# TritonDataCenter/binder

Hardware: AMD Instinct MI355X
Metric: dns_queries_per_sec (higher is better)
Workload: dtype n/a

## Files before the change

native/balancer/balancer_main.cpp:

```cpp
#include <arpa/inet.h>
#include <dirent.h>
#include <netinet/in.h>
#include <netinet/udp.h>
#include <signal.h>
#include <sys/epoll.h>
#include <sys/eventfd.h>
#include <sys/signalfd.h>
#include <sys/socket.h>
#include <sys/stat.h>
#include <sys/un.h>
#include <unistd.h>

#include <algorithm>
#include <cstdlib>
#include <cstring>
#include <map>
#include <unordered_map>
#include <chrono>
#include <memory>
#include <unordered_map>
#include <mutex>
#include <thread>
#include <set>
#include <string>
// ... 183 lines not shown
  private:
    void rescan();
    void connectBackend(Backend* be);
    void backendDown(Backend* be);
    void onBackendEvent(std::shared_ptr<Backend> be, uint32_t ev);
    void onBackendBell(std::shared_ptr<Backend> be);
    void serveBackend(Backend* be, bool fromRing);
    void offerShm(Backend* be);
    void dropShm(Backend* be);
    EventLoop::Park beforePark(bool park);
    void backendFlush(Backend* be);
    void flushToRing(Backend* be);
    Backend* pickBackend(const std::string& remoteIp);
    Backend* pickBackendFast(const struct sockaddr_storage& ss);
    Backend* chooseLeastLoaded();
    void onUdpReadable();
    Backend* routeFor(const struct sockaddr_storage& src);
    void handleUdpQuery(const uint8_t* dns, size_t dnsLen,
                        const struct sockaddr_storage& src,
                        int64_t expiry, Backend* be);
    void onTcpAccept();
    void onTcpClient(std::shared_ptr<TcpClient> c, uint32_t ev);
    void tcpClientFlush(TcpClient* c);
    void onStatsAccept();
    void sweep();
    Json snapshot() const;

    EventLoop* loop_;
    Logger log_;
    std::string host_;
    uint16_t port_;
// ... 3 lines not shown
    bool reusePort_ = false;
    int workerId_ = 0;
    int nWorkers_ = 1;

    int udpFd_ = -1, tcpFd_ = -1, statsFd_ = -1;
    std::map<std::string, std::shared_ptr<Backend>> backends_;
    std::map<int, std::shared_ptr<Backend>> backendsById_;
    std::map<std::string, int> remotes_;
    std::unordered_map<uint64_t, int> remotesFast_;
    std::map<int, std::shared_ptr<TcpClient>> tcpClients_;
    int nextBackendId_ = 1;
    int salvageDepth_ = 0;
    uint64_t udpQueries_ = 0, udpReplies_ = 0, drops_ = 0;
    uint64_t backendReads_ = 0, udpRxMsgs_ = 0;
    uint64_t shmDoorbells_ = 0, shmDrains_ = 0;

    static constexpr size_t kMaxRemotes = 262144;
    static constexpr size_t kMaxPending = 16384;
    static constexpr int64_t kReplyTtlMs = 3000;
    static constexpr int64_t kPingIntervalMs = 2000;
    static constexpr int64_t kPingTimeoutMs = 6000;

    static constexpr int kBatch = 128;
    static constexpr size_t kRxBufSz = 65536;
    std::vector<uint8_t> rxArena_ =
        std::vector<uint8_t>((size_t)kBatch * kRxBufSz);
    struct mmsghdr rxHdrs_[kBatch];
    struct iovec rxIovs_[kBatch];
    struct sockaddr_storage rxAddrs_[kBatch];
    char rxCtrl_[kBatch][CMSG_SPACE(sizeof(uint16_t))];
// ... 468 lines not shown
    if (be->fd >= 0 && be->rxShm) serveBackend(be.get(), true);
}

EventLoop::Park Balancer::beforePark(bool park) {
    EventLoop::Park out = EventLoop::Park::NoRings;
    for (auto& [id, be] : backendsById_) {
        if (!be->rxShm || be->fd < 0) continue;
        if (out == EventLoop::Park::NoRings) out = EventLoop::Park::Idle;
        if (park) {
            if (!be->shm.rx.park()) out = EventLoop::Park::Work;
        } else if (be->shm.rx.readable() != 0 || be->shm.rx.bad()) {
            serveBackend(be.get(), true);
            out = EventLoop::Park::Work;
        }
    }
    return out;
}

void Balancer::serveBackend(Backend* be, bool fromRing) {
    size_t got = 0;
    while (got < kMaxReadPerEvent) {
        if (fromRing) {
            size_t n = be->shm.rx.read(be->in.tail(kReadChunk), kReadChunk);
            if (n == 0) break;
            be->in.commit(n);
            got += n;
            backendReads_++;
            shmDrains_++;
            if (n < kReadChunk) break;
            continue;
// ... 203 lines not shown
    if (ss.ss_family == AF_INET) {
        const auto* sa = (const struct sockaddr_in*)&ss;
        inet_ntop(AF_INET, &sa->sin_addr, out, n);
        *port = ntohs(sa->sin_port);
        *family = 4;
        memcpy(addr16, &sa->sin_addr, 4);
    } else {
        const auto* sa = (const struct sockaddr_in6*)&ss;
        inet_ntop(AF_INET6, &sa->sin6_addr, out, n);
        *port = ntohs(sa->sin6_port);
        *family = 6;
        memcpy(addr16, &sa->sin6_addr, 16);
    }
}

void Balancer::onUdpReadable() {
    struct mmsghdr* hdrs = rxHdrs_;
    struct sockaddr_storage* addrs = rxAddrs_;

    while (true) {
        int n = recvmmsg(udpFd_, hdrs, kBatch, 0, nullptr);
        if (n <= 0) return;
        udpRxMsgs_ += (uint64_t)n;
        int64_t expiry = monotonicMillis() + kReplyTtlMs;
        Touched touched;
        for (int i = 0; i < n; ++i) {
            size_t seg = hdrs[i].msg_len;
            for (struct cmsghdr* cm = CMSG_FIRSTHDR(&hdrs[i].msg_hdr);
                 cm != nullptr;
                 cm = CMSG_NXTHDR(&hdrs[i].msg_hdr, cm)) {
                if (cm->cmsg_level == SOL_UDP &&
                    cm->cmsg_type == UDP_GRO) {
                    uint16_t g;
                    memcpy(&g, CMSG_DATA(cm), sizeof(g));
                    if (g > 0) seg = g;
                }
            }
            hdrs[i].msg_hdr.msg_namelen = sizeof(addrs[i]);
            hdrs[i].msg_hdr.msg_controllen = sizeof(rxCtrl_[i]);
            hdrs[i].msg_hdr.msg_flags = 0;
            Backend* be = routeFor(addrs[i]);
            const uint8_t* base = rxArena_.data() + (size_t)i * kRxBufSz;
            size_t total = hdrs[i].msg_len;
            for (size_t off = 0; off < total; off += seg) {
                size_t dnsLen = std::min(seg, total - off);
                handleUdpQuery(base + off, dnsLen, addrs[i], expiry, be);
            }
            if (be != nullptr) touch(touched, be);
        }
        flushTouched(touched);
        if (n < kBatch) return;
    }
}

void Balancer::handleUdpQuery(const uint8_t* dns, size_t dnsLen,
                              const struct sockaddr_storage& src,
                              int64_t expiry, Backend* be) {
    udpQueries_++;
    if (be == nullptr) {
        drops_++;
        return;
    }
    if (be->pendingCount > kMaxPending ||
        be->out.size() - be->outOff > (4u << 20)) {
        drops_++;
        return;
// ... 187 lines not shown
        r.set("backend", Json((int64_t)id));
        rms.push_back(std::move(r));
    }
    out.set("remotes", Json(std::move(rms)));
    out.set("udp_queries", Json((int64_t)udpQueries_));
    out.set("udp_replies", Json((int64_t)udpReplies_));
    out.set("drops", Json((int64_t)drops_));
    out.set("reply_runs", Json((int64_t)replyRuns_.runs()));
    out.set("reply_run_segments",
            Json((int64_t)replyRuns_.runSegments()));
    out.set("reply_singles", Json((int64_t)replyRuns_.singles()));
    out.set("backend_reads", Json((int64_t)backendReads_));
    out.set("udp_rx_msgs", Json((int64_t)udpRxMsgs_));
    out.set("shm_doorbells", Json((int64_t)shmDoorbells_));
    out.set("shm_drains", Json((int64_t)shmDrains_));
    return out;
}

void Balancer::onStatsAccept() {
    while (true) {
        int fd = accept4(statsFd_, nullptr, nullptr,
                         SOCK_CLOEXEC | SOCK_NONBLOCK);
        if (fd < 0) return;
        g_stats.publish(workerId_, snapshot().dump());
        std::map<std::string, Json> byPath;
        JsonArray remotes;
        int64_t udpQ = 0, udpR = 0, drops = 0;
        static const char* const kHot[] = {
            "reply_runs", "reply_run_segments", "reply_singles",
            "backend_reads", "udp_rx_msgs", "shm_doorbells",
            "shm_drains"};
        constexpr int kNHot = 7;
        int64_t hot[kNHot] = {0, 0, 0, 0, 0, 0, 0};
        JsonArray perWorker;
        int workers = 0;
        for (const std::string& frag : g_stats.all()) {
            auto parsed = Json::parse(frag);
            if (!parsed) continue;
            workers++;
            udpQ += parsed->get("udp_queries").asInt();
            udpR += parsed->get("udp_replies").asInt();
            drops += parsed->get("drops").asInt();
            Json pw = Json::object();
            pw.set("udp_queries", parsed->get("udp_queries"));
            pw.set("udp_replies", parsed->get("udp_replies"));
            pw.set("drops", parsed->get("drops"));
            for (int k = 0; k < kNHot; ++k) {
                hot[k] += parsed->get(kHot[k]).asInt();
// ... 178 lines not shown
```

native/common/loop.cpp:

```cpp
#include "loop.hpp"

#include <fcntl.h>
#include <sys/epoll.h>
#include <sys/eventfd.h>
#include <unistd.h>

#include <cstdio>
#include <cstring>
#include <stdexcept>

#include "log.hpp"

namespace bamd {

bool setNonBlocking(int fd) {
    int flags = fcntl(fd, F_GETFL, 0);
    if (flags < 0) return false;
    return fcntl(fd, F_SETFL, flags | O_NONBLOCK) == 0;
}

EventLoop::EventLoop() {
    epfd_ = epoll_create1(EPOLL_CLOEXEC);
    if (epfd_ < 0)
        throw std::runtime_error(std::string("epoll_create1: ") +
                                 strerror(errno));
    wakeFd_ = eventfd(0, EFD_NONBLOCK | EFD_CLOEXEC);
    if (wakeFd_ >= 0) {
        addFd(wakeFd_, EPOLLIN, [this](uint32_t) {
            uint64_t v;
            while (read(wakeFd_, &v, sizeof(v)) == sizeof(v)) {
            }
            std::vector<TimerCallback> tasks;
            {
                std::lock_guard<std::mutex> g(postMutex_);
                tasks.swap(posted_);
            }
            for (auto& t : tasks) t();
        });
    }
}
// ... 87 lines not shown
}

void EventLoop::runOnce(int64_t maxWaitMs) {
    std::unique_lock<std::mutex> lk;
    if (dispatchLock_ != nullptr)
        lk = std::unique_lock<std::mutex>(*dispatchLock_);
    if (!deferred_.empty()) {
        std::vector<TimerCallback> tasks;
        tasks.swap(deferred_);
        for (auto& t : tasks) t();
    }

    Park ring = beforePark_ ? beforePark_(false) : Park::NoRings;
    bool busy = ring == Park::Work;

    int64_t wait = nextTimerDelay();
    if (wait < 0 || wait > maxWaitMs) wait = maxWaitMs;
    if (ring == Park::NoRings) {
        hadWork_ = false;
    } else if (busy || hadWork_) {
        wait = 0;
    } else if (wait != 0 && beforePark_(true) == Park::Work) {
        wait = 0;
    }

    struct epoll_event evs[64];
    if (lk.owns_lock()) lk.unlock();
    int n = epoll_wait(epfd_, evs, 64, (int)wait);
    int waitErrno = errno;
    if (dispatchLock_ != nullptr) lk.lock();
    errno = waitErrno;
    hadWork_ = ring != Park::NoRings && (busy || n > 0);
    if (n < 0) {
        if (errno == EINTR) return;
        throw std::runtime_error(std::string("epoll_wait: ") +
                                 strerror(errno));
    }
    dispatching_ = true;
    for (int i = 0; i < n; ++i) {
        int fd = (int)(uint32_t)evs[i].data.u64;
        uint32_t gen = (uint32_t)(evs[i].data.u64 >> 32);
        auto it = fds_.find(fd);
        if (it == fds_.end()) continue;
        if (it->second.gen != gen) continue;
// ... 31 lines not shown
```

native/common/loop.hpp:

```cpp
#pragma once

#include <atomic>
#include <cstdint>
#include <functional>
#include <map>
#include <memory>
#include <mutex>
#include <queue>
#include <thread>
#include <vector>

namespace bamd {

class EventLoop {
  public:
    using FdCallback = std::function<void(uint32_t events)>;
    using TimerCallback = std::function<void()>;

    EventLoop();
    ~EventLoop();
    EventLoop(const EventLoop&) = delete;
    EventLoop& operator=(const EventLoop&) = delete;

    void addFd(int fd, uint32_t events, FdCallback cb);
// ... 3 lines not shown
    uint64_t addTimer(int64_t delayMs, TimerCallback cb);
    void cancelTimer(uint64_t id);

    void defer(TimerCallback cb);

    void postFromThread(TimerCallback cb);

    void run();
    void stop() { running_ = false; }
    bool running() const { return running_; }

    bool runUntil(const std::function<bool()>& pred, int64_t timeoutMs);

    void setDispatchLock(std::mutex* m) { dispatchLock_ = m; }

    enum class Park { NoRings, Idle, Work };
    using ParkHook = std::function<Park(bool park)>;
    void setBeforePark(ParkHook h) { beforePark_ = std::move(h); }

    bool inLoopThread() const {
        return loopThread_.load(std::memory_order_relaxed) ==
               std::this_thread::get_id();
    }

  private:
    void runOnce(int64_t maxWaitMs);
    void wake();
    void wakeIfForeign() {
        if (dispatchLock_ != nullptr && !inLoopThread()) wake();
    }
    int64_t nextTimerDelay() const;
    void fireTimers();

// ... 15 lines not shown
    }

    int epfd_;
    std::atomic<bool> running_{false};
    std::map<int, FdReg> fds_;
    std::vector<std::unique_ptr<FdCallback>> retired_;
    bool dispatching_ = false;
    uint32_t nextFdGen_ = 1;
    std::priority_queue<Timer, std::vector<Timer>, std::greater<Timer>> heap_;
    std::map<uint64_t, TimerCallback> timers_;
    uint64_t nextTimerId_ = 1;
    std::vector<TimerCallback> deferred_;
    ParkHook beforePark_;
    bool hadWork_ = false;

    int wakeFd_ = -1;
    std::mutex* dispatchLock_ = nullptr;
    std::atomic<std::thread::id> loopThread_{};
    std::mutex postMutex_;
    std::vector<TimerCallback> posted_;
};

bool setNonBlocking(int fd);

}
```

native/common/shmpipe.hpp:

```cpp
#pragma once

#include <fcntl.h>
#include <sys/mman.h>
#include <sys/stat.h>
#include <unistd.h>

#include <atomic>
#include <cstddef>
#include <cstdint>
#include <cstring>
#include <new>

namespace bamd::shm {

constexpr uint32_t kVersion = 1;
constexpr size_t kMinRing = 4096;
constexpr size_t kMaxRing = 64u << 20;
constexpr size_t kDefaultRing = 256u << 10;
constexpr size_t kDataOff = 4096;

struct RingCtl {
    alignas(64) std::atomic<uint64_t> tail;
    alignas(64) std::atomic<uint64_t> head;
    alignas(64) std::atomic<uint32_t> consumerParked;
// ... 10 lines not shown
inline size_t regionBytes(size_t cap) { return kDataOff + 2 * cap; }

inline void ringDoorbell(int efd) {
    uint64_t one = 1;
    ssize_t rv = ::write(efd, &one, sizeof(one));
    (void)rv;
}

class Producer {
  public:
    void attach(RingCtl* ctl, uint8_t* data, size_t cap) {
        ctl_ = ctl;
        data_ = data;
        cap_ = cap;
        tail_ = 0;
        lastHead_ = 0;
        bad_ = false;
    }
    bool bad() const { return bad_; }

    size_t write(const void* src, size_t len) {
        size_t room = space();
        if (len > room) len = room;
        if (len == 0) return 0;
        size_t off = (size_t)(tail_ & (cap_ - 1));
        size_t first = cap_ - off;
        if (first > len) first = len;
        memcpy(data_ + off, src, first);
        if (len > first)
            memcpy(data_, (const uint8_t*)src + first, len - first);
        tail_ += len;
        ctl_->tail.store(tail_, std::memory_order_release);
        return len;
    }

    bool consumerNeedsWake() {
        std::atomic_thread_fence(std::memory_order_seq_cst);
        if (ctl_->consumerParked.load(std::memory_order_relaxed) == 0)
            return false;
        return ctl_->consumerParked.exchange(
                   0, std::memory_order_acq_rel) != 0;
    }

    bool waitForSpace() {
        ctl_->producerWaiting.store(1, std::memory_order_relaxed);
        std::atomic_thread_fence(std::memory_order_seq_cst);
        if (space() == 0 && !bad_) return true;
        ctl_->producerWaiting.store(0, std::memory_order_relaxed);
// ... 4 lines not shown
    size_t space() {
        if (bad_) return 0;
        uint64_t head = ctl_->head.load(std::memory_order_acquire);
        if (head > tail_ || tail_ - head > cap_ || head < lastHead_) {
            bad_ = true;
            return 0;
        }
        lastHead_ = head;
        return cap_ - (size_t)(tail_ - head);
    }

    RingCtl* ctl_ = nullptr;
    uint8_t* data_ = nullptr;
    size_t cap_ = 0;
    uint64_t tail_ = 0;
    uint64_t lastHead_ = 0;
    bool bad_ = false;
};

class Consumer {
  public:
    void attach(RingCtl* ctl, const uint8_t* data, size_t cap) {
        ctl_ = ctl;
        data_ = data;
        cap_ = cap;
        head_ = 0;
        lastTail_ = 0;
        parked_ = false;
        bad_ = false;
    }
// ... 153 lines not shown
```

native/server/answertab.hpp:

```cpp
#pragma once

#include <cstdint>
#include <cstring>
#include <memory>

namespace bamd {

#ifdef BAMD_ANSWERTAB_TEST_HASH_MASK
inline uint64_t answertabTestHashMask = ~0ull;
#endif

class AnswerTable {
  public:
    static constexpr size_t kMaxKey = 255;
    static constexpr uint32_t kNone = 0xFFFFFFFFu;
    static constexpr size_t kMinSlots = 1024;
    static constexpr size_t kCompactMinDead = 1u << 20;
    static constexpr size_t kDefaultMaxArena = 256u << 20;

    explicit AnswerTable(size_t maxArena = kDefaultMaxArena,
                         size_t compactMinDead = kCompactMinDead)
        : maxArena_(maxArena), compactMinDead_(compactMinDead) {}

    static uint64_t hashKey(const void* key, size_t klen, uint8_t qtype) {
// ... 308 lines not shown
    memcpy(tab + 8 * n, head, headLen);
    size_t off = 0;
    for (size_t i = 0; i < n; ++i) {
        put16(tab + 8 * i, off);
        put16(tab + 8 * i + 2, seg1[i].n);
        if (seg1[i].n != 0) memcpy(segs + off, seg1[i].p, seg1[i].n);
        off += seg1[i].n;
        put16(tab + 8 * i + 4, off);
        put16(tab + 8 * i + 6, seg2[i].n);
        if (seg2[i].n != 0) memcpy(segs + off, seg2[i].p, seg2[i].n);
        off += seg2[i].n;
    }
    put16(body + 2, headLen + off);
}
inline size_t serviceMembers(const uint8_t* body) { return body[1]; }
inline size_t serviceAssemble(const uint8_t* body, const uint8_t* order,
                              uint8_t* dst) {
    size_t n = body[1];
    size_t headLen = get16(body + 4);
    const uint8_t* tab = body + 6;
    const uint8_t* head = tab + 8 * n;
    const uint8_t* segs = head + headLen;
    uint8_t* w = dst;
    memcpy(w, head, headLen);
    w += headLen;
    for (size_t i = 0; i < n; ++i) {
        const uint8_t* e = tab + 8 * order[i];
        size_t len = get16(e + 2);
        memcpy(w, segs + get16(e), len);
        w += len;
// ... 14 lines not shown
```

native/server/metrics.hpp:

```cpp
#pragma once

#include <atomic>
#include <cstdint>
#include <functional>
#include <map>
#include <memory>
#include <string>
#include <vector>

#include "../common/loop.hpp"

namespace bamd {

struct CounterShard {
    std::atomic<uint64_t> v{0};
    void bump() {
        v.store(v.load(std::memory_order_relaxed) + 1,
                std::memory_order_relaxed);
    }
    uint64_t read() const { return v.load(std::memory_order_relaxed); }
};
struct CounterFold {
    uint64_t seen = 0;
};

class Counter {
  public:
    void increment(const std::string& labels, uint64_t by = 1) {
        vals_[labels] += by;
    }
    uint64_t& slot(const std::string& labels) { return vals_[labels]; }
    void set(const std::string& labels, uint64_t v) {
        vals_[labels] = v;
    }
    const std::map<std::string, uint64_t>& values() const { return vals_; }
    void fold(const std::string& labels, const CounterShard& s,
              CounterFold& f) {
        uint64_t now = s.read();
        if (now != f.seen) vals_[labels] += now - f.seen;
        f.seen = now;
    }

  private:
    std::map<std::string, uint64_t> vals_;
};

class Histogram {
  public:
    Histogram();
    void observe(const std::string& labels, double v);

    struct Series;
    Series& seriesRef(const std::string& labels);
// ... 91 lines not shown
```

native/server/server.cpp:

```cpp
#include "server.hpp"

#include <arpa/inet.h>
#include <sched.h>
#include <sys/epoll.h>
#include <unistd.h>

#include <cstdio>
#include <cstdlib>
#include <cstring>
#include <fstream>

#include "../balancer/protocol.hpp"
#include "../common/probes.hpp"

namespace bamd {

using namespace dns;

void fillClientInfo(ClientInfo& ci, const struct sockaddr_storage& ss,
                    const char* family) {
    ci.family = family;
    if (ss.ss_family == AF_INET) {
        const auto* sa = (const struct sockaddr_in*)&ss;
        memcpy(ci.addr, &sa->sin_addr, 4);
// ... 26 lines not shown
    uint8_t head[bsock::kHeaderLen + 4];
    head[0] = bsock::kMagic;
    head[1] = bsock::FRAME_REPLY;
    head[2] = (uint8_t)plen;
    head[3] = (uint8_t)(plen >> 8);
    head[4] = (uint8_t)(plen >> 16);
    head[5] = (uint8_t)(plen >> 24);
    head[6] = (uint8_t)reqId_;
    head[7] = (uint8_t)(reqId_ >> 8);
    head[8] = (uint8_t)(reqId_ >> 16);
    head[9] = (uint8_t)(reqId_ >> 24);
    frames_->append((const char*)head, sizeof(head));
    start_ = frames_->size();
}

uint8_t* ReplySink::openWrite(size_t dnsLen) {
    if (vec_ != nullptr) {
        vec_->resize(dnsLen);
        return vec_->data();
    }
    constexpr size_t kHead = bsock::kHeaderLen + 4;
    size_t at = frames_->size();
    frames_->resize(at + kHead + dnsLen);
    uint8_t* h = (uint8_t*)frames_->data() + at;
    uint32_t plen = (uint32_t)(4 + dnsLen);
    h[0] = bsock::kMagic;
    h[1] = bsock::FRAME_REPLY;
    h[2] = (uint8_t)plen;
    h[3] = (uint8_t)(plen >> 8);
    h[4] = (uint8_t)(plen >> 16);
    h[5] = (uint8_t)(plen >> 24);
    h[6] = (uint8_t)reqId_;
    h[7] = (uint8_t)(reqId_ >> 8);
    h[8] = (uint8_t)(reqId_ >> 16);
    h[9] = (uint8_t)(reqId_ >> 24);
    start_ = at + kHead;
    return h + kHead;
}

DnsServer::DnsServer(EventLoop* loop, Logger log, ServerOptions opts,
                     Engine* engine, Collector* collector)
    : loop_(loop), log_(std::move(log)), opts_(std::move(opts)),
      engine_(engine), collector_(collector) {
    main_.loop = loop_;
    collector_->setBeforeExpose([this]() { foldShards(); });
    reqCounter_ = collector->counter("binder_requests_completed",
                                     "count of Binder requests completed");
    latHist_ = collector->histogram(
        "binder_request_latency_seconds",
        "total time to process Binder requests");
    sizeHist_ = collector->histogram("binder_response_size_bytes",
                                     "size in bytes of Binder responses");
    shmDoorbellCounter_ = collector->counter(
        "binder_balancer_shm_doorbells",
        "doorbells rung to wake a balancer across shared-memory rings");
    shmDrainCounter_ = collector->counter(
        "binder_balancer_shm_drains",
        "takes from a shared-memory query ring that returned data");

    const EngineConfig& cfg = engine_->config();
    if (!cfg.dnsDomain.empty()) dotDomain_ = "." + cfg.dnsDomain;
    dcSuffix_ = cfg.dnsDomain + "." + cfg.datacenterName;

    rxArena_.resize(kBatch * kInBuf);
    rxHdrs_.resize(kBatch);
    rxIovs_.resize(kBatch);
    rxAddrs_.resize(kBatch);
    txBufs_.resize(kBatch);
    txHdrs_.resize(kBatch);
    txIovs_.resize(kBatch);
    txAddrs_.resize(kBatch);
}

// ... 445 lines not shown
    static const std::string kA = "type=\"A\"";
    static const std::string kSrv = "type=\"SRV\"";
    auto fold = [this](ServeCtx& c) {
        reqCounter_->fold(kA, c.hits.cntA, c.folds.cntA);
        reqCounter_->fold(kSrv, c.hits.cntSrv, c.folds.cntSrv);
        latHist_->fold(kA, c.hits.latA, c.folds.latA);
        latHist_->fold(kSrv, c.hits.latSrv, c.folds.latSrv);
        sizeHist_->fold(kA, c.hits.sizeA, c.folds.sizeA);
        sizeHist_->fold(kSrv, c.hits.sizeSrv, c.folds.sizeSrv);
    };
    fold(main_);
    for (auto& c : pool_) fold(*c);
    auto foldShm = [this](ServeCtx& c) {
        shmDoorbellCounter_->fold("", c.shmDoorbells, c.shmDoorbellsFold);
        shmDrainCounter_->fold("", c.shmDrains, c.shmDrainsFold);
    };
    foldShm(main_);
    for (auto& c : pool_) foldShm(*c);
    if (queriesServed() != servedSlow_) {
        reqCounter_->slot(kA);
        reqCounter_->slot(kSrv);
        latHist_->seriesRef(kA);
        latHist_->seriesRef(kSrv);
        sizeHist_->seriesRef(kA);
        sizeHist_->seriesRef(kSrv);
    }
}

void DnsServer::serveHit(ServeCtx& ctx, const uint8_t* body, bool isSrv,
                         const uint8_t* data, ReplySink& out) {
    const size_t total = answerbody::total(body);
    uint8_t* w = out.openWrite(total);
    if (answerbody::kind(body) == answerbody::kWire) {
        memcpy(w, answerbody::wireReply(body), total);
    } else {
        size_t n = answerbody::serviceMembers(body);
        uint8_t order[answerbody::kMaxMembers];
        for (size_t i = 0; i < n; ++i) order[i] = (uint8_t)i;
        for (size_t i = n; i > 1;) {
            --i;
            size_t j = ctx.rng() % (i + 1);
            std::swap(order[i], order[j]);
        }
        answerbody::serviceAssemble(body, order, w);
    }
    w[0] = data[0];
    w[1] = data[1];
    w[2] = (uint8_t)(w[2] | (data[2] & 0x01));

    countFast(ctx, isSrv, total);
    BAMD_PROBE2("op-req-done", total, 0);
}

bool DnsServer::fastPath(ServeCtx& ctx, const uint8_t* data, size_t len,
                         bool udp, const ClientInfo& ci, ReplySink& out) {
    if (log_.enabled(LogLevel::Debug)) return false;
    FastQuery q;
    if (!parseFast(data, len, q)) return false;
    bool memo = answersOn();
    if (memo) {
        q.hash = answerHash(q);
        const uint8_t* body = ctx.answers.find(q.hash, q.isSrv ? 33 : 1,
                                               q.name, q.nlen);
// ... 1042 lines not shown
```

native/server/server.hpp:

```cpp
#pragma once

#include <netinet/in.h>
#include <sys/socket.h>
#include <sys/un.h>

#include <atomic>
#include <functional>
#include <random>
#include <map>
#include <memory>
#include <mutex>
#include <string>
#include <thread>
#include <vector>

#include "../common/log.hpp"
#include "../common/loop.hpp"
#include "../common/shmpipe.hpp"
#include "../engine/engine.hpp"
#include "answertab.hpp"
#include "framebuf.hpp"
#include "metrics.hpp"

namespace bamd {
// ... 20 lines not shown
    uint8_t ipFamily = 0;
    uint16_t port = 0;
    const char* family = "udp";

    const char* address(char (&buf)[48]) const;
};

class ReplySink {
  public:
    explicit ReplySink(std::vector<uint8_t>* v) : vec_(v) {}
    ReplySink(std::string* frames, uint32_t reqId)
        : frames_(frames), reqId_(reqId) {}

    void open(size_t dnsLen);
    uint8_t* openWrite(size_t dnsLen);
    void append(const uint8_t* p, size_t n) {
        if (vec_ != nullptr)
            vec_->insert(vec_->end(), p, p + n);
        else
            frames_->append((const char*)p, n);
    }
    uint8_t* dns() {
        return vec_ != nullptr ? vec_->data()
                               : (uint8_t*)frames_->data() + start_;
    }
    size_t dnsLen() const {
        return vec_ != nullptr ? vec_->size() : frames_->size() - start_;
    }
    std::vector<uint8_t>* vec() { return vec_; }

// ... 131 lines not shown
        CounterFold cntA, cntSrv;
        Histogram::Fold latA, latSrv, sizeA, sizeSrv;
    };
    void countFast(ServeCtx& ctx, bool isSrv, size_t bytes);
    void foldShards();

    struct alignas(64) ServeCtx {
        AnswerTable answers;
        std::mt19937 rng{std::random_device{}()};
        HitShards hits;
        EventLoop* loop = nullptr;
        std::map<int, std::shared_ptr<BalConn>> balConns;
        std::vector<BalConn*> shmConns;
        CounterShard shmDoorbells, shmDrains;
        CounterFold shmDoorbellsFold, shmDrainsFold;
        bool pooled = false;

        std::atomic<uint64_t> inboxSeq{0};
        uint64_t inboxSeen = 0;
        std::mutex inboxMu;
        std::vector<std::string> inbox;

        HitFolds folds;

        std::unique_ptr<EventLoop> ownLoop;
        std::thread thread;
    };
    void postInvalidate(ServeCtx& ctx, std::string_view domain);
    void drainInbox(ServeCtx& ctx) {
        if (ctx.inboxSeq.load(std::memory_order_acquire) != ctx.inboxSeen)
// ... 47 lines not shown
    void sweepIdleTcp();
    void balFlush(ServeCtx& ctx, BalConn* c);
    void closeTcp(TcpConn* c);
    void closeBal(ServeCtx& ctx, BalConn* c);

    EventLoop* loop_;
    Logger log_;
    ServerOptions opts_;
    Engine* engine_;
    Collector* collector_;
    RecursionIface* recursion_ = nullptr;

    Counter* reqCounter_ = nullptr;
    Counter* shmDoorbellCounter_ = nullptr;
    Counter* shmDrainCounter_ = nullptr;
    Histogram* latHist_ = nullptr;
    Histogram* sizeHist_ = nullptr;

    int udpFd_ = -1;
    int tcpFd_ = -1;
    int balFd_ = -1;
    uint16_t boundPort_ = 0;
    uint64_t servedSlow_ = 0;

    std::map<int, std::shared_ptr<TcpConn>> tcpConns_;

    static constexpr int kBatch = 64;
    static constexpr size_t kInBuf = 4096;
    std::vector<uint8_t> rxArena_;
    std::vector<struct mmsghdr> rxHdrs_;
// ... 13 lines not shown
```

Before: 24.16 million.

## Skip redundant epoll polls in busy loops and poll UDP from ring hook

The event loop now skips the epoll_wait call on busy rounds for up to a configurable number of rounds within the same millisecond, which cuts empty zero-timeout syscalls. The balancer's park hook also does one recvmmsg pass when rings had work, so UDP input is drained without waiting for epoll. The server writes wire answers with a single append instead of resize+memcpy, and takes the flags byte from the cached body rather than reading it back. The shm producer gains reserve/commit/publish helpers, and loop statistics counters are added. The trade-off is that fd events can be noticed slightly later, and the hot path now does extra atomic counter updates.

After: 23.26 million. 3.7% lower.

```diff
diff --git a/native/balancer/balancer_main.cpp b/native/balancer/balancer_main.cpp
--- a/native/balancer/balancer_main.cpp
+++ b/native/balancer/balancer_main.cpp
@@ -221,7 +221,7 @@
     Backend* pickBackend(const std::string& remoteIp);
     Backend* pickBackendFast(const struct sockaddr_storage& ss);
     Backend* chooseLeastLoaded();
-    void onUdpReadable();
+    void onUdpReadable(bool once = false);
     Backend* routeFor(const struct sockaddr_storage& src);
     void handleUdpQuery(const uint8_t* dns, size_t dnsLen,
                         const struct sockaddr_storage& src,
@@ -255,6 +255,7 @@
     uint64_t udpQueries_ = 0, udpReplies_ = 0, drops_ = 0;
     uint64_t backendReads_ = 0, udpRxMsgs_ = 0;
     uint64_t shmDoorbells_ = 0, shmDrains_ = 0;
+    uint64_t udpRecvCalls_ = 0, udpRecvEmpty_ = 0;
 
     static constexpr size_t kMaxRemotes = 262144;
     static constexpr size_t kMaxPending = 16384;
@@ -753,6 +754,8 @@
             out = EventLoop::Park::Work;
         }
     }
+    if (park || out == EventLoop::Park::NoRings) return out;
+    if (out == EventLoop::Park::Work) onUdpReadable(true);
     return out;
 }
 
@@ -986,13 +989,17 @@
     }
 }
 
-void Balancer::onUdpReadable() {
+void Balancer::onUdpReadable(bool once) {
     struct mmsghdr* hdrs = rxHdrs_;
     struct sockaddr_storage* addrs = rxAddrs_;
 
     while (true) {
         int n = recvmmsg(udpFd_, hdrs, kBatch, 0, nullptr);
-        if (n <= 0) return;
+        udpRecvCalls_++;
+        if (n <= 0) {
+            udpRecvEmpty_++;
+            return;
+        }
         udpRxMsgs_ += (uint64_t)n;
         int64_t expiry = monotonicMillis() + kReplyTtlMs;
         Touched touched;
@@ -1021,7 +1028,7 @@
             if (be != nullptr) touch(touched, be);
         }
         flushTouched(touched);
-        if (n < kBatch) return;
+        if (n < kBatch || once) return;
     }
 }
 
@@ -1239,6 +1246,14 @@
     out.set("udp_rx_msgs", Json((int64_t)udpRxMsgs_));
     out.set("shm_doorbells", Json((int64_t)shmDoorbells_));
     out.set("shm_drains", Json((int64_t)shmDrains_));
+    EventLoop::Stats ls = loop_->stats();
+    out.set("epoll_waits", Json((int64_t)ls.waits));
+    out.set("epoll_zero_waits", Json((int64_t)ls.zeroWaits));
+    out.set("epoll_empty_polls", Json((int64_t)ls.emptyPolls));
+    out.set("loop_parks", Json((int64_t)ls.parks));
+    out.set("loop_skipped_looks", Json((int64_t)ls.skipped));
+    out.set("udp_recv_calls", Json((int64_t)udpRecvCalls_));
+    out.set("udp_recv_empty", Json((int64_t)udpRecvEmpty_));
     return out;
 }
 
@@ -1254,9 +1269,11 @@
         static const char* const kHot[] = {
             "reply_runs", "reply_run_segments", "reply_singles",
             "backend_reads", "udp_rx_msgs", "shm_doorbells",
-            "shm_drains"};
-        constexpr int kNHot = 7;
-        int64_t hot[kNHot] = {0, 0, 0, 0, 0, 0, 0};
+            "shm_drains", "epoll_waits", "epoll_zero_waits",
+            "epoll_empty_polls", "loop_parks", "loop_skipped_looks",
+            "udp_recv_calls", "udp_recv_empty"};
+        constexpr int kNHot = sizeof(kHot) / sizeof(kHot[0]);
+        int64_t hot[kNHot] = {};
         JsonArray perWorker;
         int workers = 0;
         for (const std::string& frag : g_stats.all()) {
diff --git a/native/common/loop.cpp b/native/common/loop.cpp
--- a/native/common/loop.cpp
+++ b/native/common/loop.cpp
@@ -6,6 +6,7 @@
 #include <unistd.h>
 
 #include <cstdio>
+#include <cstdlib>
 #include <cstring>
 #include <stdexcept>
 
@@ -24,6 +25,10 @@
     if (epfd_ < 0)
         throw std::runtime_error(std::string("epoll_create1: ") +
                                  strerror(errno));
+    if (const char* e = getenv("BINDER_LOOP_BUSY_ROUNDS")) {
+        int n = atoi(e);
+        if (n >= 1 && n <= 64) busyRounds_ = n;
+    }
     wakeFd_ = eventfd(0, EFD_NONBLOCK | EFD_CLOEXEC);
     if (wakeFd_ >= 0) {
         addFd(wakeFd_, EPOLLIN, [this](uint32_t) {
@@ -141,6 +146,16 @@
     Park ring = beforePark_ ? beforePark_(false) : Park::NoRings;
     bool busy = ring == Park::Work;
 
+    if (busy && dispatchLock_ == nullptr &&
+        ++sinceLook_ < busyRounds_ && monotonicMillis() == lastLookMs_) {
+        bump(skipped_);
+        hadWork_ = true;
+        fireTimers();
+        return;
+    }
+    sinceLook_ = 0;
+    lastLookMs_ = monotonicMillis();
+
     int64_t wait = nextTimerDelay();
     if (wait < 0 || wait > maxWaitMs) wait = maxWaitMs;
     if (ring == Park::NoRings) {
@@ -153,8 +168,14 @@
 
     struct epoll_event evs[64];
     if (lk.owns_lock()) lk.unlock();
+    bump(waits_);
+    if (wait == 0)
+        bump(zeroWaits_);
+    else
+        bump(parks_);
     int n = epoll_wait(epfd_, evs, 64, (int)wait);
     int waitErrno = errno;
+    if (wait == 0 && n == 0) bump(emptyPolls_);
     if (dispatchLock_ != nullptr) lk.lock();
     errno = waitErrno;
     hadWork_ = ring != Park::NoRings && (busy || n > 0);
diff --git a/native/common/loop.hpp b/native/common/loop.hpp
--- a/native/common/loop.hpp
+++ b/native/common/loop.hpp
@@ -41,9 +41,26 @@
 
     void setDispatchLock(std::mutex* m) { dispatchLock_ = m; }
 
+    static constexpr int kBusyRounds = 2;
+    void setBusyRounds(int n) { busyRounds_ = n < 1 ? 1 : n; }
     enum class Park { NoRings, Idle, Work };
     using ParkHook = std::function<Park(bool park)>;
     void setBeforePark(ParkHook h) { beforePark_ = std::move(h); }
+
+    struct Stats {
+        uint64_t waits = 0;
+        uint64_t zeroWaits = 0;
+        uint64_t emptyPolls = 0;
+        uint64_t parks = 0;
+        uint64_t skipped = 0;
+    };
+    Stats stats() const {
+        return {waits_.load(std::memory_order_relaxed),
+                zeroWaits_.load(std::memory_order_relaxed),
+                emptyPolls_.load(std::memory_order_relaxed),
+                parks_.load(std::memory_order_relaxed),
+                skipped_.load(std::memory_order_relaxed)};
+    }
 
     bool inLoopThread() const {
         return loopThread_.load(std::memory_order_relaxed) ==
@@ -89,6 +106,16 @@
     ParkHook beforePark_;
     bool hadWork_ = false;
 
+    static void bump(std::atomic<uint64_t>& c) {
+        c.store(c.load(std::memory_order_relaxed) + 1,
+                std::memory_order_relaxed);
+    }
+    std::atomic<uint64_t> waits_{0}, zeroWaits_{0}, emptyPolls_{0},
+        parks_{0}, skipped_{0};
+    int busyRounds_ = kBusyRounds;
+    int sinceLook_ = 0;
+    int64_t lastLookMs_ = -1;
+
     int wakeFd_ = -1;
     std::mutex* dispatchLock_ = nullptr;
     std::atomic<std::thread::id> loopThread_{};
diff --git a/native/common/loop_check_main.cpp b/native/common/loop_check_main.cpp
--- /dev/null
+++ b/native/common/loop_check_main.cpp
@@ -0,0 +1,217 @@
+#include <sys/epoll.h>
+#include <sys/resource.h>
+#include <time.h>
+#include <unistd.h>
+
+#include <atomic>
+#include <chrono>
+#include <cstdio>
+#include <cstdlib>
+#include <functional>
+#include <mutex>
+#include <thread>
+
+#include "log.hpp"
+#include "loop.hpp"
+
+using bamd::EventLoop;
+
+static int g_failed = 0;
+#define CHECK(cond, ...)                                            \
+    do {                                                            \
+        if (!(cond)) {                                              \
+            fprintf(stderr, "FAIL %s:%d: %s: ", __FILE__, __LINE__, \
+                    #cond);                                         \
+            fprintf(stderr, __VA_ARGS__);                           \
+            fprintf(stderr, "\n");                                  \
+            g_failed++;                                             \
+        }                                                           \
+    } while (0)
+
+static int64_t nowUs() {
+    struct timespec ts;
+    clock_gettime(CLOCK_MONOTONIC, &ts);
+    return (int64_t)ts.tv_sec * 1000000 + ts.tv_nsec / 1000;
+}
+
+static int64_t cpuUs() {
+    struct rusage ru;
+    getrusage(RUSAGE_SELF, &ru);
+    return (int64_t)(ru.ru_utime.tv_sec + ru.ru_stime.tv_sec) * 1000000 +
+           ru.ru_utime.tv_usec + ru.ru_stime.tv_usec;
+}
+
+static void checkFdWithinBusyRounds() {
+    EventLoop loop;
+    int p[2];
+    if (pipe(p) != 0) abort();
+    uint64_t rounds = 0, armedAt = 0, seenAt = 0;
+    int armed = 0;
+    uint64_t worst = 0;
+    loop.setBeforePark([&](bool) {
+        rounds++;
+        if (!armed && rounds % 7 == 3) {
+            char c = 'x';
+            if (write(p[1], &c, 1) != 1) abort();
+            armed = 1;
+            armedAt = rounds;
+        }
+        return EventLoop::Park::Work;
+    });
+    int hits = 0;
+    loop.addFd(p[0], EPOLLIN, [&](uint32_t) {
+        char c;
+        if (read(p[0], &c, 1) != 1) abort();
+        seenAt = rounds;
+        uint64_t d = seenAt - armedAt;
+        if (d > worst) worst = d;
+        armed = 0;
+        hits++;
+    });
+    loop.runUntil([&] { return hits >= 200; }, 5000);
+    CHECK(hits >= 200, "only %d dispatches", hits);
+    CHECK(worst < (uint64_t)EventLoop::kBusyRounds,
+          "fd waited %llu rounds", (unsigned long long)worst);
+    EventLoop::Stats st = loop.stats();
+    CHECK(st.skipped > 0, "nothing was skipped");
+    CHECK(st.parks == 0, "a busy loop parked %llu times",
+          (unsigned long long)st.parks);
+    printf("fd: worst %llu rounds, %llu waits, %llu skipped\n",
+           (unsigned long long)worst, (unsigned long long)st.waits,
+           (unsigned long long)st.skipped);
+    close(p[0]);
+    close(p[1]);
+}
+
+static void checkTimerUnderLoad() {
+    EventLoop loop;
+    loop.setBeforePark([](bool) { return EventLoop::Park::Work; });
+    int64_t worst = 0;
+    int fired = 0;
+    int64_t t0 = 0;
+    std::function<void()> arm = [&] {
+        t0 = nowUs();
+        loop.addTimer(1, [&] {
+            int64_t d = nowUs() - t0;
+            if (d > worst) worst = d;
+            if (++fired < 50) arm();
+        });
+    };
+    arm();
+    loop.runUntil([&] { return fired >= 50; }, 5000);
+    CHECK(fired >= 50, "only %d timers", fired);
+    CHECK(worst <= 2000, "1 ms timer took %lld us", (long long)worst);
+    printf("timer: worst %lld us\n", (long long)worst);
+}
+
+static void checkIdleBlocks() {
+    EventLoop loop;
+    uint64_t parkCalls = 0;
+    loop.setBeforePark([&](bool park) {
+        if (park) parkCalls++;
+        return EventLoop::Park::Idle;
+    });
+    int64_t c0 = cpuUs();
+    bool done = false;
+    loop.addTimer(200, [&] { done = true; });
+    loop.runUntil([&] { return done; }, 2000);
+    int64_t cpu = cpuUs() - c0;
+    EventLoop::Stats st = loop.stats();
+    CHECK(st.waits <= 12, "%llu epoll_wait calls in 200 ms idle",
+          (unsigned long long)st.waits);
+    CHECK(st.parks >= 4, "%llu parks", (unsigned long long)st.parks);
+    CHECK(st.skipped == 0, "idle loop skipped");
+    CHECK(parkCalls == st.parks, "hook(true) %llu times, %llu parks",
+          (unsigned long long)parkCalls, (unsigned long long)st.parks);
+    CHECK(cpu < 20000, "%lld us of CPU while idle", (long long)cpu);
+    printf("idle: %llu waits, %llu parks, %lld us cpu\n",
+           (unsigned long long)st.waits, (unsigned long long)st.parks,
+           (long long)cpu);
+}
+
+static void checkDispatchLock() {
+    EventLoop loop;
+    std::mutex mu;
+    loop.setDispatchLock(&mu);
+    std::atomic<uint64_t> rounds{0};
+    loop.setBeforePark([&](bool) {
+        rounds.fetch_add(1, std::memory_order_relaxed);
+        int64_t until = nowUs() + 20;
+        while (nowUs() < until) {
+        }
+        return EventLoop::Park::Work;
+    });
+    std::atomic<bool> stop{false};
+    int trials = 0, within = 0;
+    uint64_t worst = 0;
+    std::thread other([&] {
+        while (rounds.load() < 10) std::this_thread::yield();
+        for (; trials < 50; ++trials) {
+            uint64_t r0 = rounds.load(std::memory_order_relaxed);
+            while (!mu.try_lock()) {
+            }
+            uint64_t d = rounds.load(std::memory_order_relaxed) - r0;
+            mu.unlock();
+            if (d <= 1) within++;
+            if (d > worst) worst = d;
+            int64_t until = nowUs() + 7 + trials % 13;
+            while (nowUs() < until) {
+            }
+        }
+        stop = true;
+    });
+    loop.runUntil([&] { return stop.load(); }, 10000);
+    other.join();
+    EventLoop::Stats st = loop.stats();
+    CHECK(stop.load(), "lock taker never finished");
+    CHECK(st.skipped == 0, "a loop with a dispatch lock skipped %llu",
+          (unsigned long long)st.skipped);
+    CHECK(within >= 45, "lock within one round in %d of %d (worst %llu)",
+          within, trials, (unsigned long long)worst);
+    printf("lock: within one round %d/%d, worst %llu\n", within, trials,
+           (unsigned long long)worst);
+}
+
+static void checkNoRingsUnchanged() {
+    for (int withHook = 0; withHook < 2; ++withHook) {
+        EventLoop loop;
+        uint64_t rounds = 0;
+        if (withHook)
+            loop.setBeforePark([&](bool) {
+                rounds++;
+                return EventLoop::Park::NoRings;
+            });
+        int fired = 0;
+        std::function<void()> arm = [&] {
+            loop.addTimer(1, [&] {
+                if (++fired < 20) arm();
+            });
+        };
+        arm();
+        loop.runUntil([&] { return fired >= 20; }, 2000);
+        EventLoop::Stats st = loop.stats();
+        CHECK(fired >= 20, "timers");
+        CHECK(st.skipped == 0, "skipped without rings");
+        if (withHook)
+            CHECK(st.waits == rounds, "%llu waits in %llu rounds",
+                  (unsigned long long)st.waits,
+                  (unsigned long long)rounds);
+        CHECK(st.waits < 200, "%llu waits for 20 ms of timers",
+              (unsigned long long)st.waits);
+    }
+    printf("norings: ok\n");
+}
+
+int main() {
+    checkFdWithinBusyRounds();
+    checkTimerUnderLoad();
+    checkIdleBlocks();
+    checkDispatchLock();
+    checkNoRingsUnchanged();
+    if (g_failed != 0) {
+        fprintf(stderr, "%d check(s) failed\n", g_failed);
+        return 1;
+    }
+    printf("loop check OK\n");
+    return 0;
+}
diff --git a/native/common/shmpipe.hpp b/native/common/shmpipe.hpp
--- a/native/common/shmpipe.hpp
+++ b/native/common/shmpipe.hpp
@@ -48,6 +48,7 @@
         data_ = data;
         cap_ = cap;
         tail_ = 0;
+        published_ = 0;
         lastHead_ = 0;
         bad_ = false;
     }
@@ -64,8 +65,21 @@
         if (len > first)
             memcpy(data_, (const uint8_t*)src + first, len - first);
         tail_ += len;
+        publish();
+        return len;
+    }
+
+    uint8_t* reserve(size_t n) {
+        if (n == 0 || n > space()) return nullptr;
+        size_t off = (size_t)(tail_ & (cap_ - 1));
+        if (n > cap_ - off) return nullptr;
+        return data_ + off;
+    }
+    void commit(size_t n) { tail_ += n; }
+    bool unpublished() const { return tail_ != published_; }
+    void publish() {
+        published_ = tail_;
         ctl_->tail.store(tail_, std::memory_order_release);
-        return len;
     }
 
     bool consumerNeedsWake() {
@@ -100,6 +114,7 @@
     uint8_t* data_ = nullptr;
     size_t cap_ = 0;
     uint64_t tail_ = 0;
+    uint64_t published_ = 0;
     uint64_t lastHead_ = 0;
     bool bad_ = false;
 };
diff --git a/native/common/shmpipe_reserve_check_main.cpp b/native/common/shmpipe_reserve_check_main.cpp
--- /dev/null
+++ b/native/common/shmpipe_reserve_check_main.cpp
@@ -0,0 +1,342 @@
+#include <poll.h>
+#include <sys/eventfd.h>
+
+#include <cstdio>
+#include <cstdlib>
+#include <deque>
+#include <memory>
+#include <random>
+#include <thread>
+#include <vector>
+
+#include "shmpipe.hpp"
+
+using namespace bamd;
+
+namespace {
+
+std::atomic<int> g_failures{0};
+
+#define CHECK(cond)                                                    \
+    do {                                                               \
+        if (!(cond)) {                                                 \
+            fprintf(stderr, "FAIL %s:%d: %s\n", __FILE__, __LINE__,    \
+                    #cond);                                            \
+            g_failures++;                                              \
+        }                                                              \
+    } while (0)
+
+constexpr size_t kCap = 4096;
+constexpr int kWaitMs = 10000;
+
+inline uint8_t streamByte(uint64_t i) {
+    return (uint8_t)((i * 2654435761u) >> 11);
+}
+
+struct HeapRing {
+    std::unique_ptr<shm::RingCtl> ctl{new shm::RingCtl};
+    std::unique_ptr<uint8_t[]> data{new uint8_t[kCap]};
+    shm::Producer tx;
+    shm::Consumer rx;
+    HeapRing() {
+        ctl->tail.store(0);
+        ctl->head.store(0);
+        ctl->consumerParked.store(0);
+        ctl->producerWaiting.store(0);
+        memset(data.get(), 0xEE, kCap);
+        tx.attach(ctl.get(), data.get(), kCap);
+        rx.attach(ctl.get(), data.get(), kCap);
+    }
+    void advanceTo(uint64_t at) {
+        std::vector<uint8_t> junk(kCap);
+        uint64_t pos = 0;
+        while (pos < at) {
+            size_t n = (size_t)std::min<uint64_t>(at - pos, kCap);
+            CHECK(tx.write(junk.data(), n) == n);
+            CHECK(rx.read(junk.data(), n) == n);
+            pos += n;
+        }
+    }
+};
+
+void caseModel(unsigned seed, int frames) {
+    HeapRing r;
+    std::mt19937 rng(seed);
+    std::deque<uint8_t> model;
+    uint64_t produced = 0, consumed = 0;
+    size_t pending = 0;
+    int byReserve = 0, byWrite = 0, refusedWrap = 0, refusedFull = 0;
+    std::vector<uint8_t> buf(kCap);
+    for (int f = 0; f < frames; ++f) {
+        size_t n = 1 + rng() % 300;
+        bool viaReserve = rng() % 3 != 0;
+        size_t used = (size_t)(produced - consumed);
+        size_t off = (size_t)(produced & (kCap - 1));
+        if (viaReserve) {
+            uint8_t* p = r.tx.reserve(n);
+            bool fits = n <= kCap - used, flat = n <= kCap - off;
+            CHECK((p != nullptr) == (fits && flat));
+            if (p == nullptr) {
+                if (!fits) refusedFull++;
+                else refusedWrap++;
+                viaReserve = false;
+            } else {
+                CHECK(p == r.data.get() + off);
+                for (size_t i = 0; i < n; ++i)
+                    p[i] = streamByte(produced + i);
+                r.tx.commit(n);
+                produced += n;
+                pending += n;
+                byReserve++;
+                CHECK(r.rx.readable() == model.size());
+                if (rng() % 4 == 0) {
+                    r.tx.publish();
+                    for (size_t i = 0; i < pending; ++i)
+                        model.push_back(
+                            streamByte(produced - pending + i));
+                    pending = 0;
+                    CHECK(r.rx.readable() == model.size());
+                }
+            }
+        }
+        if (!viaReserve) {
+            for (size_t i = 0; i < n; ++i)
+                buf[i] = streamByte(produced + i);
+            size_t took = r.tx.write(buf.data(), n);
+            CHECK(took == std::min(n, kCap - used));
+            if (took != 0) {
+                for (size_t i = 0; i < pending + took; ++i)
+                    model.push_back(streamByte(produced - pending + i));
+                pending = 0;
+                byWrite++;
+            }
+            produced += took;
+            CHECK(r.rx.readable() == model.size());
+        }
+        if (pending != 0 && kCap - (produced - consumed) < 300) {
+            r.tx.publish();
+            for (size_t i = 0; i < pending; ++i)
+                model.push_back(streamByte(produced - pending + i));
+            pending = 0;
+        }
+        CHECK(r.tx.unpublished() == (pending != 0));
+        if (rng() % 3 == 0) {
+            size_t want = 1 + rng() % 800;
+            size_t got = r.rx.read(buf.data(), want);
+            CHECK(got == std::min(want, model.size()));
+            for (size_t i = 0; i < got; ++i) {
+                CHECK(buf[i] == model.front());
+                CHECK(buf[i] == streamByte(consumed + i));
+                model.pop_front();
+            }
+            consumed += got;
+        }
+    }
+    r.tx.publish();
+    CHECK(!r.tx.bad() && !r.rx.bad());
+    CHECK(byReserve > frames / 4 && byWrite > 0);
+    CHECK(refusedWrap > 0 && refusedFull > 0);
+    printf("model: %d frames, %d reserved, %d written, refused %d at the "
+           "wrap, %d for room\n", frames, byReserve, byWrite, refusedWrap,
+           refusedFull);
+}
+
+void caseEdges() {
+    {
+        HeapRing r;
+        r.advanceTo(kCap - 100);
+        uint8_t* p = r.tx.reserve(100);
+        CHECK(p == r.data.get() + kCap - 100);
+        if (p) memset(p, 0x11, 100);
+        r.tx.commit(100);
+        uint8_t* q = r.tx.reserve(50);
+        CHECK(q == r.data.get());
+        if (q) memset(q, 0x22, 50);
+        r.tx.commit(50);
+        CHECK(r.rx.readable() == 0);
+        r.tx.publish();
+        uint8_t out[150];
+        CHECK(r.rx.read(out, 150) == 150);
+        CHECK(out[0] == 0x11 && out[99] == 0x11 && out[100] == 0x22 &&
+              out[149] == 0x22);
+    }
+    {
+        HeapRing r;
+        r.advanceTo(kCap - 100);
+        CHECK(r.tx.reserve(101) == nullptr);
+        CHECK(!r.tx.bad());
+        uint8_t src[101];
+        memset(src, 0x33, sizeof(src));
+        CHECK(r.tx.write(src, 101) == 101);
+        uint8_t out[101];
+        CHECK(r.rx.read(out, 101) == 101);
+        CHECK(out[0] == 0x33 && out[100] == 0x33);
+    }
+    {
+        HeapRing r;
+        std::vector<uint8_t> fill(kCap - 64, 0x44);
+        CHECK(r.tx.write(fill.data(), fill.size()) == fill.size());
+        uint8_t* p = r.tx.reserve(64);
+        CHECK(p == r.data.get() + kCap - 64);
+        CHECK(r.tx.reserve(65) == nullptr);
+        r.tx.commit(64);
+        CHECK(r.tx.reserve(1) == nullptr);
+        r.tx.publish();
+        CHECK(r.rx.readable() == kCap);
+    }
+    {
+        HeapRing r;
+        std::vector<uint8_t> fill(kCap - 63, 0x55);
+        CHECK(r.tx.write(fill.data(), fill.size()) == fill.size());
+        CHECK(r.tx.reserve(64) == nullptr);
+        CHECK(r.tx.reserve(63) != nullptr);
+        CHECK(!r.tx.bad());
+        uint8_t one;
+        CHECK(r.rx.read(&one, 1) == 1);
+        CHECK(r.tx.reserve(64) == nullptr);
+        CHECK(r.tx.reserve(63) != nullptr);
+    }
+    CHECK(HeapRing().tx.reserve(kCap + 1) == nullptr);
+    printf("edges: ok\n");
+}
+
+void caseBadHead() {
+    {
+        HeapRing r;
+        r.ctl->head.store(1);
+        CHECK(r.tx.reserve(10) == nullptr);
+        CHECK(r.tx.bad());
+        uint8_t b[4] = {0};
+        CHECK(r.tx.write(b, 4) == 0);
+        r.ctl->head.store(0);
+        CHECK(r.tx.reserve(10) == nullptr);
+    }
+    {
+        HeapRing r;
+        r.advanceTo(1000);
+        CHECK(r.tx.reserve(10) != nullptr);
+        r.ctl->head.store(500);
+        CHECK(r.tx.reserve(10) == nullptr);
+        CHECK(r.tx.bad());
+    }
+    {
+        HeapRing r;
+        r.advanceTo(3 * kCap);
+        r.tx.attach(r.ctl.get(), r.data.get(), kCap);
+        CHECK(r.tx.reserve(10) == nullptr);
+        CHECK(r.tx.bad());
+    }
+    {
+        HeapRing r;
+        CHECK(r.tx.reserve(100) != nullptr);
+        r.tx.commit(100);
+        r.ctl->head.store(50);
+        uint8_t* p = r.tx.reserve(100);
+        CHECK(p == nullptr || p == r.data.get() + 100);
+        r.ctl->head.store(200);
+        CHECK(r.tx.reserve(10) == nullptr);
+        CHECK(r.tx.bad());
+    }
+    printf("bad head: ok\n");
+}
+
+bool waitBell(int efd) {
+    struct pollfd p = {efd, POLLIN, 0};
+    if (poll(&p, 1, kWaitMs) <= 0) return false;
+    uint64_t v;
+    ssize_t n = read(efd, &v, sizeof(v));
+    (void)n;
+    return true;
+}
+
+void caseThreads(unsigned seed, int frames) {
+    HeapRing r;
+    int bellToC = eventfd(0, EFD_NONBLOCK | EFD_CLOEXEC);
+    int bellToP = eventfd(0, EFD_NONBLOCK | EFD_CLOEXEC);
+    CHECK(bellToC >= 0 && bellToP >= 0);
+    std::atomic<bool> lost{false};
+    std::atomic<uint64_t> total{0};
+    std::atomic<bool> done{false};
+
+    std::thread producer([&]() {
+        std::mt19937 rng(seed);
+        std::vector<uint8_t> buf(300);
+        uint64_t sent = 0;
+        int batch = 0;
+        for (int f = 0; f < frames && !lost; ++f) {
+            size_t n = 1 + rng() % 300;
+            uint8_t* p = r.tx.reserve(n);
+            if (p != nullptr) {
+                for (size_t i = 0; i < n; ++i) p[i] = streamByte(sent + i);
+                r.tx.commit(n);
+            } else {
+                for (size_t i = 0; i < n; ++i)
+                    buf[i] = streamByte(sent + i);
+                size_t off = 0;
+                while (off < n && !lost) {
+                    size_t k = r.tx.write(buf.data() + off, n - off);
+                    off += k;
+                    if (k != 0 && r.tx.consumerNeedsWake())
+                        shm::ringDoorbell(bellToC);
+                    if (off < n && r.tx.waitForSpace() &&
+                        !waitBell(bellToP))
+                        lost = true;
+                }
+            }
+            sent += n;
+            if (++batch >= 8 || f + 1 == frames) {
+                batch = 0;
+                if (r.tx.unpublished()) r.tx.publish();
+                if (r.tx.consumerNeedsWake()) shm::ringDoorbell(bellToC);
+            }
+        }
+        total = sent;
+        done = true;
+        shm::ringDoorbell(bellToC);
+        CHECK(!r.tx.bad());
+    });
+    std::thread consumer([&]() {
+        std::mt19937 rng(seed + 7);
+        std::vector<uint8_t> buf(2000);
+        uint64_t seen = 0, wrong = 0;
+        while (!lost) {
+            size_t n = r.rx.read(buf.data(), 1 + rng() % 2000);
+            if (n == 0) {
+                if (done && seen == total) break;
+                if (r.rx.park() && !done && !waitBell(bellToC))
+                    lost = true;
+                continue;
+            }
+            for (size_t i = 0; i < n; ++i)
+                if (buf[i] != streamByte(seen + i)) wrong++;
+            seen += n;
+            if (r.rx.producerNeedsWake()) shm::ringDoorbell(bellToP);
+        }
+        CHECK(wrong == 0);
+        CHECK(seen == total);
+        CHECK(!r.rx.bad());
+    });
+    producer.join();
+    consumer.join();
+    CHECK(!lost);
+    close(bellToC);
+    close(bellToP);
+    printf("threads: %llu bytes\n", (unsigned long long)total.load());
+}
+
+}
+
+int main(int argc, char** argv) {
+    unsigned seed = argc > 1 ? (unsigned)atoi(argv[1]) : 1;
+    int frames = argc > 2 ? atoi(argv[2]) : 100000;
+    caseModel(seed, frames);
+    caseEdges();
+    caseBadHead();
+    caseThreads(seed, frames);
+    if (g_failures != 0) {
+        fprintf(stderr, "%d failure(s)\n", g_failures.load());
+        return 1;
+    }
+    printf("shmpipe reserve check OK\n");
+    return 0;
+}
diff --git a/native/server/answertab.hpp b/native/server/answertab.hpp
--- a/native/server/answertab.hpp
+++ b/native/server/answertab.hpp
@@ -346,6 +346,10 @@
     put16(body + 2, headLen + off);
 }
 inline size_t serviceMembers(const uint8_t* body) { return body[1]; }
+inline uint8_t flagsByte(const uint8_t* body) {
+    return body[0] == kWire ? body[4 + 2]
+                            : body[6 + 8 * (size_t)body[1] + 2];
+}
 inline size_t serviceAssemble(const uint8_t* body, const uint8_t* order,
                               uint8_t* dst) {
     size_t n = body[1];
diff --git a/native/server/metrics.hpp b/native/server/metrics.hpp
--- a/native/server/metrics.hpp
+++ b/native/server/metrics.hpp
@@ -36,7 +36,9 @@
     const std::map<std::string, uint64_t>& values() const { return vals_; }
     void fold(const std::string& labels, const CounterShard& s,
               CounterFold& f) {
-        uint64_t now = s.read();
+        fold(labels, s.read(), f);
+    }
+    void fold(const std::string& labels, uint64_t now, CounterFold& f) {
         if (now != f.seen) vals_[labels] += now - f.seen;
         f.seen = now;
     }
diff --git a/native/server/server.cpp b/native/server/server.cpp
--- a/native/server/server.cpp
+++ b/native/server/server.cpp
@@ -64,15 +64,9 @@
     start_ = frames_->size();
 }
 
-uint8_t* ReplySink::openWrite(size_t dnsLen) {
-    if (vec_ != nullptr) {
-        vec_->resize(dnsLen);
-        return vec_->data();
-    }
-    constexpr size_t kHead = bsock::kHeaderLen + 4;
-    size_t at = frames_->size();
-    frames_->resize(at + kHead + dnsLen);
-    uint8_t* h = (uint8_t*)frames_->data() + at;
+namespace {
+constexpr size_t kReplyHead = bsock::kHeaderLen + 4;
+inline void replyHead(uint8_t* h, size_t dnsLen, uint32_t reqId) {
     uint32_t plen = (uint32_t)(4 + dnsLen);
     h[0] = bsock::kMagic;
     h[1] = bsock::FRAME_REPLY;
@@ -80,12 +74,37 @@
     h[3] = (uint8_t)(plen >> 8);
     h[4] = (uint8_t)(plen >> 16);
     h[5] = (uint8_t)(plen >> 24);
-    h[6] = (uint8_t)reqId_;
-    h[7] = (uint8_t)(reqId_ >> 8);
-    h[8] = (uint8_t)(reqId_ >> 16);
-    h[9] = (uint8_t)(reqId_ >> 24);
-    start_ = at + kHead;
-    return h + kHead;
+    h[6] = (uint8_t)reqId;
+    h[7] = (uint8_t)(reqId >> 8);
+    h[8] = (uint8_t)(reqId >> 16);
+    h[9] = (uint8_t)(reqId >> 24);
+}
+}
+
+uint8_t* ReplySink::openWrite(size_t dnsLen) {
+    if (vec_ != nullptr) {
+        vec_->resize(dnsLen);
+        return vec_->data();
+    }
+    size_t at = frames_->size();
+    frames_->resize(at + kReplyHead + dnsLen);
+    uint8_t* h = (uint8_t*)frames_->data() + at;
+    replyHead(h, dnsLen, reqId_);
+    start_ = at + kReplyHead;
+    return h + kReplyHead;
+}
+
+uint8_t* ReplySink::put(const uint8_t* dns, size_t n) {
+    if (vec_ != nullptr) {
+        vec_->assign(dns, dns + n);
+        return vec_->data();
+    }
+    uint8_t head[kReplyHead];
+    replyHead(head, n, reqId_);
+    frames_->append((const char*)head, sizeof(head));
+    start_ = frames_->size();
+    frames_->append((const char*)dns, n);
+    return (uint8_t*)frames_->data() + start_;
 }
 
 DnsServer::DnsServer(EventLoop* loop, Logger log, ServerOptions opts,
@@ -107,6 +126,21 @@
     shmDrainCounter_ = collector->counter(
         "binder_balancer_shm_drains",
         "takes from a shared-memory query ring that returned data");
+    loopWaitCounter_ = collector->counter(
+        "binder_loop_epoll_waits",
+        "epoll_wait calls made by the serving loops");
+    loopZeroWaitCounter_ = collector->counter(
+        "binder_loop_epoll_zero_waits",
+        "epoll_wait calls made with a zero timeout");
+    loopEmptyPollCounter_ = collector->counter(
+        "binder_loop_epoll_empty_polls",
+        "zero-timeout epoll_wait calls that returned no event");
+    loopParkCounter_ = collector->counter(
+        "binder_loop_parks",
+        "blocking waits entered by the serving loops");
+    loopSkipCounter_ = collector->counter(
+        "binder_loop_skipped_looks",
+        "busy rounds of the serving loops that did not ask epoll");
 
     const EngineConfig& cfg = engine_->config();
     if (!cfg.dnsDomain.empty()) dotDomain_ = "." + cfg.dnsDomain;
@@ -582,6 +616,13 @@
     auto foldShm = [this](ServeCtx& c) {
         shmDoorbellCounter_->fold("", c.shmDoorbells, c.shmDoorbellsFold);
         shmDrainCounter_->fold("", c.shmDrains, c.shmDrainsFold);
+        if (c.loop == nullptr) return;
+        EventLoop::Stats ls = c.loop->stats();
+        loopWaitCounter_->fold("", ls.waits, c.loopFolds[0]);
+        loopZeroWaitCounter_->fold("", ls.zeroWaits, c.loopFolds[1]);
+        loopEmptyPollCounter_->fold("", ls.emptyPolls, c.loopFolds[2]);
+        loopParkCounter_->fold("", ls.parks, c.loopFolds[3]);
+        loopSkipCounter_->fold("", ls.skipped, c.loopFolds[4]);
     };
     foldShm(main_);
     for (auto& c : pool_) foldShm(*c);
@@ -598,10 +639,11 @@
 void DnsServer::serveHit(ServeCtx& ctx, const uint8_t* body, bool isSrv,
                          const uint8_t* data, ReplySink& out) {
     const size_t total = answerbody::total(body);
-    uint8_t* w = out.openWrite(total);
+    uint8_t* w;
     if (answerbody::kind(body) == answerbody::kWire) {
-        memcpy(w, answerbody::wireReply(body), total);
+        w = out.put(answerbody::wireReply(body), total);
     } else {
+        w = out.openWrite(total);
         size_t n = answerbody::serviceMembers(body);
         uint8_t order[answerbody::kMaxMembers];
         for (size_t i = 0; i < n; ++i) order[i] = (uint8_t)i;
@@ -614,7 +656,7 @@
     }
     w[0] = data[0];
     w[1] = data[1];
-    w[2] = (uint8_t)(w[2] | (data[2] & 0x01));
+    w[2] = (uint8_t)(answerbody::flagsByte(body) | (data[2] & 0x01));
 
     countFast(ctx, isSrv, total);
     BAMD_PROBE2("op-req-done", total, 0);
diff --git a/native/server/server.hpp b/native/server/server.hpp
--- a/native/server/server.hpp
+++ b/native/server/server.hpp
@@ -58,6 +58,7 @@
 
     void open(size_t dnsLen);
     uint8_t* openWrite(size_t dnsLen);
+    uint8_t* put(const uint8_t* dns, size_t n);
     void append(const uint8_t* p, size_t n) {
         if (vec_ != nullptr)
             vec_->insert(vec_->end(), p, p + n);
@@ -219,6 +220,7 @@
         std::vector<BalConn*> shmConns;
         CounterShard shmDoorbells, shmDrains;
         CounterFold shmDoorbellsFold, shmDrainsFold;
+        CounterFold loopFolds[5];
         bool pooled = false;
 
         std::atomic<uint64_t> inboxSeq{0};
@@ -296,6 +298,11 @@
     Counter* reqCounter_ = nullptr;
     Counter* shmDoorbellCounter_ = nullptr;
     Counter* shmDrainCounter_ = nullptr;
+    Counter* loopWaitCounter_ = nullptr;
+    Counter* loopZeroWaitCounter_ = nullptr;
+    Counter* loopEmptyPollCounter_ = nullptr;
+    Counter* loopParkCounter_ = nullptr;
+    Counter* loopSkipCounter_ = nullptr;
     Histogram* latHist_ = nullptr;
     Histogram* sizeHist_ = nullptr;
 
```
